# NikNazarov/TorchPIV

Hardware: AMD Instinct MI355X
Metric: image-pairs/sec at 4 MP, wind=64 ov=32 2-pass CWS; % HBM roofline (higher is better)
Workload: dtype u32 exact sums + f64 / f32

## Files before the change

torchpiv_amd/csrc/xcorr_tile.hpp:

```cpp
#pragma once
#include <hip/hip_runtime.h>
#include <stdint.h>
#include <stdlib.h>

#include "fft_inreg.hpp"
#include "piv_kernels.h"

namespace tpiv {

template <int WS, bool PLANAR_ = false>
struct TileGeo {
    static constexpr int WPW = 64 / WS;
    static constexpr int TS = WS > 32 ? 32 : WS;
    static constexpr int PITCH = TS + 1;
    static constexpr int NT = 64 / TS;
    static constexpr int TILE = TS * PITCH;
    static constexpr bool PLANAR = PLANAR_;
    static constexpr int HROWS = WS / 2 + 1;
    static constexpr int HTILE = HROWS * PITCH;
    static constexpr int LDS_FLOATS = NT * TILE * (PLANAR ? 1 : 2);
    static constexpr int MAP_PITCH = WS + 1;
    static constexpr int NDW = WS / 4;
};

// ... 84 lines not shown
template <int K, int N>
__device__ __forceinline__ float byte_f(const uint32_t (&d)[N]) {
    return (float)((d[K >> 2] >> (8 * (K & 3))) & 0xffu);
}

#ifndef TPIV_SDWA_LERP
#define TPIV_SDWA_LERP 0
#endif
constexpr float SDWA_UP = 0x1p125f, SDWA_DN = 0x1p-24f, SDWA_INV = 0x1p24f;
template <int K, int N>
__device__ __forceinline__ float byte_d(const uint32_t (&d)[N]) {
    return __uint_as_float((d[K >> 2] >> (8 * (K & 3))) & 0xffu);
}

template <int N>
__device__ __forceinline__ void load_dwords(const uint8_t* __restrict__ p, uint32_t (&d)[N]) {
    __builtin_memcpy(&d[0], p, 4 * N);
}

__device__ __forceinline__ float bilerp_ref(float f11, float f21, float f12, float f22, float wx_up,
                                            float wx_dn, float wy_up, float wy_dn, bool degenerate) {
#pragma clang fp contract(off)
    float r = (f11 * wx_up) * wy_up;
    r = r + (f21 * wx_dn) * wy_up;
    r = r + (f12 * wx_up) * wy_dn;
    r = r + (f22 * wx_dn) * wy_dn;
    return degenerate ? f11 : r;
}

__device__ __forceinline__ float bilerp_ref_m(float f11, float f21, float f12, float f22, float wx_up,
                                              float wx_dn, float wy_up, float wy_dn, unsigned degenerate_mask) {
#pragma clang fp contract(off)
    float r = (f11 * wx_up) * wy_up;
    r = r + (f21 * wx_dn) * wy_up;
    r = r + (f12 * wx_up) * wy_dn;
    r = r + (f22 * wx_dn) * wy_dn;
    const unsigned bits = (degenerate_mask & __float_as_uint(f11)) | (~degenerate_mask & __float_as_uint(r));
    return __uint_as_float(bits);
}

#ifdef TPIV_STAMPS
#define TPIV_STAMP_DECL unsigned long long st_acc[16] = {}; unsigned long long st_prev = 0; unsigned st_iter = 0; \
    unsigned long long st_t0 = __builtin_amdgcn_s_memtime(), st_r0 = __builtin_amdgcn_s_memrealtime();
#define TPIV_STAMP_START                                                                  \
    do {                                                                                  \
        __builtin_amdgcn_sched_barrier(0);                                                \
        asm volatile("s_memtime %0\n\ts_waitcnt lgkmcnt(0)" : "=s"(st_prev)::"memory");    \
        __builtin_amdgcn_sched_barrier(0);                                                \
    } while (0)
#define TPIV_STAMP(i)                                                                     \
    do {                                                                                  \
        unsigned long long st_t;                                                          \
        __builtin_amdgcn_sched_barrier(0);                                                \
        asm volatile("s_memtime %0\n\ts_waitcnt lgkmcnt(0)" : "=s"(st_t)::"memory");       \
        __builtin_amdgcn_sched_barrier(0);                                                \
        st_acc[i] += st_t - st_prev;                                                      \
        st_prev = st_t;                                                                   \
    } while (0)
#define TPIV_STAMP_FLUSH(pp)                                                              \
    do {                                                                                  \
        if ((pp).stamps != nullptr && threadIdx.x == 0) {                                 \
            for (int q_ = 0; q_ < 16; ++q_) atomicAdd(&(pp).stamps[q_], st_acc[q_]);      \
            atomicAdd(&(pp).stamps[16], (unsigned long long)st_iter);                     \
            atomicAdd(&(pp).stamps[17], __builtin_amdgcn_s_memtime() - st_t0);            \
            atomicAdd(&(pp).stamps[18], __builtin_amdgcn_s_memrealtime() - st_r0);        \
        }                                                                                 \
    } while (0)
#else
#define TPIV_STAMP_DECL
#define TPIV_STAMP_START
#define TPIV_STAMP(i)
#define TPIV_STAMP_FLUSH(pp)
#endif

__device__ __forceinline__ int fast_div(int n, unsigned magic, int shift) {
    return (int)(((unsigned long long)(unsigned)n * magic) >> shift);
}
inline void fast_div_setup(unsigned d, unsigned& magic, int& shift) {
    int s_ = 0;
    while ((1ull << s_) < d) ++s_;
    shift = 31 + s_;
    magic = (unsigned)(((1ull << shift) + d - 1) / d);
}

__device__ __forceinline__ int fresh_lane() {
    int l = (int)__builtin_amdgcn_mbcnt_hi(~0u, __builtin_amdgcn_mbcnt_lo(~0u, 0u));
    asm volatile("" : "+v"(l));
    return l;
}

__device__ __forceinline__ void wave_sync() {
    __builtin_amdgcn_fence(__ATOMIC_ACQ_REL, "wavefront");
    __builtin_amdgcn_wave_barrier();
}

template <int WS, bool DIGITREV, bool PLANAR>
__device__ __forceinline__ void transpose_tile(cf (&a)[WS], float* lds, int lane) {
    using G = TileGeo<WS, PLANAR>;
    constexpr int P = G::PITCH;
    cf* tile = reinterpret_cast<cf*>(lds);
    if constexpr (PLANAR && WS > 32) {
        static_for<0, 32>([&](auto kc) TPIV_LAMBDA_INLINE {
            constexpr int k = decltype(kc)::value;
            constexpr int lo = DIGITREV ? FFT_POS<k, WS> : k;
            constexpr int hi = DIGITREV ? FFT_POS<k + 32, WS> : k + 32;
            auto rx = __builtin_amdgcn_permlane32_swap(__float_as_uint(a[lo].x), __float_as_uint(a[hi].x),
                                                       false, false);
            auto ry = __builtin_amdgcn_permlane32_swap(__float_as_uint(a[lo].y), __float_as_uint(a[hi].y),
                                                       false, false);
            a[lo].x = __uint_as_float(rx[0]);
            a[hi].x = __uint_as_float(rx[1]);
            a[lo].y = __uint_as_float(ry[0]);
            a[hi].y = __uint_as_float(ry[1]);
        });
        float* t = lds + (lane >> 5) * G::TILE;
        const int i = lane & 31;
        auto plane = [&](auto comp) TPIV_LAMBDA_INLINE {
            constexpr bool Y = decltype(comp)::value;
            float lowhalf[32];
            wave_sync();
            static_for<0, 32>([&](auto kc) TPIV_LAMBDA_INLINE {
                constexpr int k = decltype(kc)::value;
                constexpr int src = DIGITREV ? FFT_POS<k, WS> : k;
                t[i * P + k] = Y ? a[src].y : a[src].x;
            });
            wave_sync();
#pragma unroll
            for (int r = 0; r < 32; ++r) lowhalf[r] = t[r * P + i];
            wave_sync();
            static_for<0, 32>([&](auto kc) TPIV_LAMBDA_INLINE {
                constexpr int k = decltype(kc)::value;
                constexpr int src = DIGITREV ? FFT_POS<k + 32, WS> : k + 32;
                t[i * P + k] = Y ? a[src].y : a[src].x;
            });
            wave_sync();
#pragma unroll
            for (int r = 0; r < 32; ++r) {
                if constexpr (Y) {
                    a[32 + r].y = t[r * P + i];
                    a[r].y = lowhalf[r];
                } else {
                    a[32 + r].x = t[r * P + i];
                    a[r].x = lowhalf[r];
                }
            }
        };
        plane(std::false_type{});
        plane(std::true_type{});
    } else if constexpr (PLANAR) {
        float* t = lds + (lane / WS) * G::TILE;
        const int i = lane % WS;
        wave_sync();
        static_for<0, WS>([&](auto kc) TPIV_LAMBDA_INLINE {
            constexpr int k = decltype(kc)::value;
            constexpr int src = DIGITREV ? FFT_POS<k, WS> : k;
            t[i * P + k] = a[src].x;
        });
        wave_sync();
#pragma unroll
        for (int r = 0; r < WS; ++r) a[r].x = t[r * P + i];
        wave_sync();
        static_for<0, WS>([&](auto kc) TPIV_LAMBDA_INLINE {
            constexpr int k = decltype(kc)::value;
            constexpr int src = DIGITREV ? FFT_POS<k, WS> : k;
            t[i * P + k] = a[src].y;
        });
        wave_sync();
#pragma unroll
        for (int r = 0; r < WS; ++r) a[r].y = t[r * P + i];
    } else if constexpr (WS <= 32) {
        cf* t = tile + (lane / WS) * G::TILE;
        const int i = lane % WS;
        wave_sync();
        static_for<0, WS>([&](auto kc) TPIV_LAMBDA_INLINE {
            constexpr int k = decltype(kc)::value;
            constexpr int src = DIGITREV ? FFT_POS<k, WS> : k;
            t[i * P + k] = a[src];
        });
        wave_sync();
#pragma unroll
        for (int r = 0; r < WS; ++r) a[r] = t[r * P + i];
    } else {
        static_for<0, 32>([&](auto kc) TPIV_LAMBDA_INLINE {
            constexpr int k = decltype(kc)::value;
            constexpr int lo = DIGITREV ? FFT_POS<k, WS> : k;
            constexpr int hi = DIGITREV ? FFT_POS<k + 32, WS> : k + 32;
            auto rx = __builtin_amdgcn_permlane32_swap(__float_as_uint(a[lo].x), __float_as_uint(a[hi].x),
                                                       false, false);
            auto ry = __builtin_amdgcn_permlane32_swap(__float_as_uint(a[lo].y), __float_as_uint(a[hi].y),
                                                       false, false);
            a[lo].x = __uint_as_float(rx[0]);
            a[hi].x = __uint_as_float(rx[1]);
            a[lo].y = __uint_as_float(ry[0]);
            a[hi].y = __uint_as_float(ry[1]);
        });
        cf* t = tile + (lane >> 5) * G::TILE;
        const int i = lane & 31;
        cf lowhalf[32];
        wave_sync();
        static_for<0, 32>([&](auto kc) TPIV_LAMBDA_INLINE {
            constexpr int k = decltype(kc)::value;
            constexpr int src = DIGITREV ? FFT_POS<k, WS> : k;
            t[i * P + k] = a[src];
        });
        wave_sync();
#pragma unroll
        for (int r = 0; r < 32; ++r) lowhalf[r] = t[r * P + i];
        wave_sync();
        static_for<0, 32>([&](auto kc) TPIV_LAMBDA_INLINE {
            constexpr int k = decltype(kc)::value;
            constexpr int src = DIGITREV ? FFT_POS<k + 32, WS> : k + 32;
            t[i * P + k] = a[src];
        });
        wave_sync();
#pragma unroll
        for (int r = 0; r < 32; ++r) a[32 + r] = t[r * P + i];
#pragma unroll
        for (int r = 0; r < 32; ++r) a[r] = lowhalf[r];
    }
}

template <int WS, bool PLANAR>
__device__ __forceinline__ void transpose_half(const cf (&a)[WS], cf (&g)[WS / 2 + 1], float* lds, int lane) {
    static_assert(WS <= 32 || WS == 64, "one tile per window");
    using G = TileGeo<WS, PLANAR>;
    constexpr int P = G::PITCH, M = WS / 2;
    const int i = lane % WS;
    if constexpr (WS == 64) {
        constexpr int Q = M + 1;
        static_assert(WS * Q * (PLANAR ? 1 : 2) <= G::LDS_FLOATS, "half-spectrum plane fits the tile");
        cf b[WS];
        static_for<0, WS>([&](auto kc) TPIV_LAMBDA_INLINE {
            constexpr int k = decltype(kc)::value;
            b[k] = a[FFT_POS<k, WS>];
            asm volatile("" : "+v"(b[k].x), "+v"(b[k].y));
        });
        wave_sync();
        if constexpr (!PLANAR) {
            cf* t = reinterpret_cast<cf*>(lds);
            if (i <= M) {
                static_for<0, WS>([&](auto kc) TPIV_LAMBDA_INLINE {
                    constexpr int k = decltype(kc)::value;
                    t[k * Q + i] = b[k];
                });
            }
            wave_sync();
#pragma unroll
            for (int r = 0; r <= M; ++r) g[r] = t[i * Q + r];
        } else {
        if (i <= M) {
            static_for<0, WS>([&](auto kc) TPIV_LAMBDA_INLINE {
                constexpr int k = decltype(kc)::value;
                lds[k * Q + i] = b[k].x;
            });
        }
        wave_sync();
#pragma unroll
        for (int r = 0; r <= M; ++r) g[r].x = lds[i * Q + r];
        wave_sync();
        if (i <= M) {
            static_for<0, WS>([&](auto kc) TPIV_LAMBDA_INLINE {
                constexpr int k = decltype(kc)::value;
                lds[k * Q + i] = b[k].y;
            });
        }
        wave_sync();
#pragma unroll
        for (int r = 0; r <= M; ++r) g[r].y = lds[i * Q + r];
        }
    } else if constexpr (PLANAR) {
        float* t = lds + (lane / WS) * G::HTILE;
        wave_sync();
        if (i <= M) {
            static_for<0, WS>([&](auto kc) TPIV_LAMBDA_INLINE {
                constexpr int k = decltype(kc)::value;
                t[i * P + k] = a[FFT_POS<k, WS>].x;
            });
        }
        wave_sync();
#pragma unroll
        for (int r = 0; r <= M; ++r) g[r].x = t[r * P + i];
        wave_sync();
        if (i <= M) {
            static_for<0, WS>([&](auto kc) TPIV_LAMBDA_INLINE {
                constexpr int k = decltype(kc)::value;
                t[i * P + k] = a[FFT_POS<k, WS>].y;
            });
        }
        wave_sync();
#pragma unroll
        for (int r = 0; r <= M; ++r) g[r].y = t[r * P + i];
    } else {
        cf* t = reinterpret_cast<cf*>(lds) + (lane / WS) * G::HTILE;
        wave_sync();
        if (i <= M) {
            static_for<0, WS>([&](auto kc) TPIV_LAMBDA_INLINE {
                constexpr int k = decltype(kc)::value;
                t[i * P + k] = a[FFT_POS<k, WS>];
            });
        }
        wave_sync();
#pragma unroll
        for (int r = 0; r <= M; ++r) g[r] = t[r * P + i];
    }
}

struct ItemGeom {
    int pair, win, y0, x0;
    int active;
    size_t fidx;
};

#ifndef TPIV_COOP1
#define TPIV_COOP1 0
#endif
template <int WS>
struct Coop1 {
    static constexpr bool ON = TPIV_COOP1 && (WS == 64 || WS == 32);
    static constexpr int P16 = WS / 16;
    static constexpr int PITCH4 = WS / 16 + 1;
};
template <int WS, int MODE>
struct RawRows;
template <int WS>
struct RawRows<WS, MODE_PASS1> {
    uint32_t a[WS / 4], b[WS / 4];
};
template <int WS>
struct RawRows<WS, MODE_DWS> {
    uint32_t a[WS / 4], b[WS / 4];
    long long qa, qb;
    int reg;
    int cls;
    int fix;
};
template <int WS>
struct CoopGeo {
#ifndef TPIV_COOP
#define TPIV_COOP 1
#endif
    static constexpr bool ON = TPIV_COOP && (WS == 16 || WS == 32 || WS == 64);
    static constexpr int NROW = WS + 1;
    static constexpr int RPG = (WS + 1 + 15) / 16;
    static constexpr int LOADED = 16 * RPG;
    static constexpr int T = NROW * RPG;
    static constexpr int NCH = (T + WS - 1) / WS;
    static constexpr int PITCH4 = RPG | 1;
    static constexpr int PATCH4 = NROW * PITCH4;
    static constexpr int BLOCK4 = (2 * PATCH4 + 15) / 16 * 16;
    static constexpr int FLOATS = (64 / WS) * BLOCK4 * 4;
    static constexpr int LDS_FLOATS = FLOATS + (64 / WS) * (WS + 1) * 4;
    static_assert(!ON || RPG <= PITCH4, "patch row pitch");
    __device__ static __forceinline__ void chunk(int ci, int& j, int& part) {
        if constexpr (RPG == 2) {
            j = ci >> 1;
            part = ci & 1;
        } else if constexpr (RPG == 3) {
            j = (ci * 171) >> 9;
            part = ci - 3 * j;
        } else {
            static_assert(RPG == 5, "chunks per row");
            j = (ci * 205) >> 10;
            part = ci - 5 * j;
        }
    }
};
template <int WS>
struct CoopOff {
    int o[CoopGeo<WS>::ON ? CoopGeo<WS>::NCH : 1];
    __device__ __forceinline__ void init(int r, int W) {
        if constexpr (CoopGeo<WS>::ON) {
#pragma unroll
            for (int k = 0; k < CoopGeo<WS>::NCH; ++k) {
                int j, part;
                CoopGeo<WS>::chunk(r + WS * k, j, part);
                o[k] = r + WS * k < CoopGeo<WS>::T ? j * W + 16 * part : 0;
            }
        }
    }
};
template <int WS>
struct RawRows<WS, MODE_CWS> {
    static constexpr int NB = WS / 4 + 1;
    uint32_t a0[CoopGeo<WS>::ON ? 1 : NB], a1[CoopGeo<WS>::ON ? 1 : NB], b0[CoopGeo<WS>::ON ? 1 : NB], b1[CoopGeo<WS>::ON ? 1 : NB];
    uint32_t ca[CoopGeo<WS>::ON ? CoopGeo<WS>::NCH : 1][4], cb[CoopGeo<WS>::ON ? CoopGeo<WS>::NCH : 1][4];
    int reg;
    int cls;
    int fix;
};

struct CwsRow {
    float wya_up, wya_dn, wyb_up, wyb_dn;
    int dya, uya, dyb, uyb;
    int ydeg_a, ydeg_b;
};
__device__ __forceinline__ CwsRow cws_row(int gy, float vy) {
    CwsRow c;
    const float gyf = (float)gy;
    const float nya = gyf - vy, nyb = gyf + vy;
    const float uya_f = ceilf(nya), dya_f = floorf(nya);
    const float uyb_f = ceilf(nyb), dyb_f = floorf(nyb);
    c.uya = f2i_sat_t(uya_f);
    c.dya = f2i_sat_t(dya_f);
    c.uyb = f2i_sat_t(uyb_f);
    c.dyb = f2i_sat_t(dyb_f);
    c.wya_up = uya_f - nya;
    c.wya_dn = nya - dya_f;
    c.wyb_up = uyb_f - nyb;
    c.wyb_dn = nyb - dyb_f;
    c.ydeg_a = c.uya == c.dya;
    c.ydeg_b = c.uyb == c.dyb;
    return c;
}

__device__ __forceinline__ int classify_row(long long q, int used, int loaded, int HW, long long& qload) {
    const long long lim = (long long)HW - loaded;
    if (q >= 0 && q <= lim) {
        qload = q;
        return 0;
    }
    if (q + used - 1 <= 0) {
        qload = 0;
        return 1;
    }
    if (q >= (long long)HW - 1) {
        qload = lim;
        return 2;
    }
    qload = 0;
    return 3;
}

__device__ __forceinline__ int clamp_i(int v, int lo, int hi) { return v < lo ? lo : (v > hi ? hi : v); }

__device__ __forceinline__ int classify_row32(int q, int used, int loaded, int HW, int& qload) {
    const int lim = HW - loaded;
    const bool inside = (unsigned)q <= (unsigned)lim;
    const bool before = q + used - 1 <= 0;
    const bool behind = q >= HW - 1;
    qload = inside ? q : (behind && !before ? lim : 0);
    return inside ? 0 : (before ? 1 : (behind ? 2 : 3));
}

template <int N>
__device__ __forceinline__ void fix_row(uint32_t (&d)[N], int cls) {
    const uint32_t px = (cls == 1 ? (d[0] & 0xffu) : (d[N - 1] >> 24)) * 0x01010101u;
#pragma unroll
    for (int i = 0; i < N; ++i) d[i] = cls != 0 ? px : d[i];
}
template <int N>
__device__ __forceinline__ void fix_row(uint32_t (&d)[N], int cls, uint32_t last) {
    const uint32_t px = (cls == 1 ? (d[0] & 0xffu) : (last >> 24)) * 0x01010101u;
#pragma unroll
    for (int i = 0; i < N; ++i) d[i] = cls != 0 ? px : d[i];
}

template <int WS, int MODE, bool FAST = false>
__device__ __forceinline__ void issue_rows(const PassParams& p, const ItemGeom& g, int r, float vx, float vy,
                                           RawRows<WS, MODE>& raw, const CoopOff<WS>& coff) {
    const int HW = p.H * p.W;
    const uint8_t* __restrict__ fa = p.A + (size_t)g.pair * HW;
    const uint8_t* __restrict__ fb = p.B + (size_t)g.pair * HW;
    const long long base = (long long)(g.y0 + r) * p.W + g.x0;
    if constexpr (MODE == MODE_PASS1) {
        if constexpr (Coop1<WS>::ON) {
            using C1 = Coop1<WS>;
            const unsigned o0 = (unsigned)(g.y0 * p.W + g.x0);
#pragma unroll
            for (int k = 0; k < C1::P16; ++k) {
                const int ci = r + WS * k, j = ci / C1::P16, part = ci % C1::P16;
                const unsigned o_ = o0 + (unsigned)(j * p.W + 16 * part);
                load_dwords<4>(fa + o_, *reinterpret_cast<uint32_t(*)[4]>(&raw.a[4 * k]));
                load_dwords<4>(fb + o_, *reinterpret_cast<uint32_t(*)[4]>(&raw.b[4 * k]));
            }
        } else {
#ifdef TPIV_EXP_P1LOADS
            load_dwords<4 * TPIV_EXP_P1LOADS>(fa + base, *reinterpret_cast<uint32_t(*)[4 * TPIV_EXP_P1LOADS]>(&raw.a[0]));
            load_dwords<4 * TPIV_EXP_P1LOADS>(fb + base, *reinterpret_cast<uint32_t(*)[4 * TPIV_EXP_P1LOADS]>(&raw.b[0]));
#pragma unroll
            for (int k = 4 * TPIV_EXP_P1LOADS; k < WS / 4; ++k) {
                raw.a[k] = 0x11213141u * (unsigned)(r + 1 + k);
                raw.b[k] = 0x31112141u * (unsigned)(r + 3 + k);
            }
#else
            load_dwords<WS / 4>(fa + base, raw.a);
            load_dwords<WS / 4>(fb + base, raw.b);
#endif
        }
    } else if constexpr (MODE == MODE_DWS) {
        const long long sh = (long long)vy * p.W + (long long)vx;
        raw.qa = base - sh;
        raw.qb = base + sh;
        long long la, lb;
        const int ca = classify_row(raw.qa, WS, WS, HW, la), cb = classify_row(raw.qb, WS, WS, HW, lb);
        raw.reg = __all(ca != 3 && cb != 3) ? 1 : 0;
        raw.cls = ca | (cb << 2);
        raw.fix = (raw.reg && __any(raw.cls != 0)) ? 1 : 0;
        load_dwords<WS / 4>(fa + (raw.reg ? la : base), raw.a);
        load_dwords<WS / 4>(fb + (raw.reg ? lb : base), raw.b);
    } else {
        constexpr int NB = WS / 4 + 1;
        const CwsRow c = cws_row(g.y0 + r, vy);
        const float fvx = floorf(vx);
        const int W_ = p.W;
        const int ivx = clamp_i(f2i_sat_t(fvx), -W_, W_);
        const int rlo = -8, rhi = p.H + 7;
        const int dya = clamp_i(c.dya, rlo, rhi), uya = clamp_i(c.uya, rlo, rhi);
        const int dyb = clamp_i(c.dyb, rlo, rhi), uyb = clamp_i(c.uyb, rlo, rhi);
        const int xa = g.x0 - ivx - 1, xb = g.x0 + ivx;
        const int qa0 = dya * W_ + xa, qa1 = uya * W_ + xa;
        const int qb0 = dyb * W_ + xb, qb1 = uyb * W_ + xb;
        using CG = CoopGeo<WS>;
        constexpr int LOADED = CG::ON ? CG::LOADED : 4 * NB;
        const float gxr = (float)(g.x0 + r);
        const float nxa_r = gxr - vx, nxb_r = gxr + vx;
        const float fxa_r = floorf(nxa_r), fxb_r = floorf(nxb_r);
        const bool col_ok = fxa_r == (float)(g.x0 + r - ivx - 1) && fxb_r == (float)(g.x0 + r + ivx) &&
                            fxa_r != nxa_r && fxb_r != nxb_r;
        bool reg = col_ok && fabsf(vx) < (float)p.W && !(FAST && (c.ydeg_a | c.ydeg_b));
        int la0 = 0, la1 = 0, lb0 = 0, lb1 = 0, cls = 0;
        auto classify_own = [&]() TPIV_LAMBDA_INLINE {
            const int c0 = classify_row32(qa0, WS + 1, LOADED, HW, la0), c1 = classify_row32(qa1, WS + 1, LOADED, HW, la1);
            const int c2 = classify_row32(qb0, WS + 1, LOADED, HW, lb0), c3 = classify_row32(qb1, WS + 1, LOADED, HW, lb1);
            reg = reg && c0 != 3 && c1 != 3 && c2 != 3 && c3 != 3;
            cls = c0 | (c1 << 2) | (c2 << 4) | (c3 << 6);
        };
        if constexpr (CG::ON) {
            const float gy0f = (float)g.y0;
            const int base_a = clamp_i(f2i_sat_t(floorf(gy0f - vy)), rlo, rhi);
            const int base_b = clamp_i(f2i_sat_t(floorf(gy0f + vy)), rlo, rhi);
            reg = reg && (unsigned)(dya - base_a) <= (unsigned)WS && (unsigned)(uya - base_a) <= (unsigned)WS &&
                  (unsigned)(dyb - base_b) <= (unsigned)WS && (unsigned)(uyb - base_b) <= (unsigned)WS;
            const bool inside = base_a >= 0 && base_a + WS < p.H && base_b >= 0 && base_b + WS < p.H &&
                                xa >= 0 && xa + LOADED <= W_ && xb >= 0 && xb + LOADED <= W_;
            const bool all_in = __all(inside);
            if (!all_in) classify_own();
            raw.reg = __all(reg) ? 1 : 0;
            raw.cls = cls;
            raw.fix = (raw.reg && __any(raw.cls != 0)) ? 1 : 0;
            unsigned oa[CG::NCH], ob[CG::NCH];
            if (all_in) {
                const int qa_o = base_a * W_ + xa, qb_o = base_b * W_ + xb;
#pragma unroll
                for (int k = 0; k < CG::NCH; ++k) {
                    oa[k] = (unsigned)(qa_o + coff.o[k]);
                    ob[k] = (unsigned)(qb_o + coff.o[k]);
                }
            } else {
#pragma unroll
                for (int k = 0; k < CG::NCH; ++k) {
                    const int ci = r + WS * k;
                    int j, part;
                    CG::chunk(ci, j, part);
                    int qa_l, qb_l;
                    const int ra = clamp_i(base_a + j, rlo, rhi), rb = clamp_i(base_b + j, rlo, rhi);
                    classify_row32(ra * W_ + xa, WS + 1, LOADED, HW, qa_l);
                    classify_row32(rb * W_ + xb, WS + 1, LOADED, HW, qb_l);
                    const bool live = ci < CG::T;
                    oa[k] = live ? (unsigned)(qa_l + 16 * part) : 0u;
                    ob[k] = live ? (unsigned)(qb_l + 16 * part) : 0u;
                }
            }
#pragma unroll
            for (int k = 0; k < CG::NCH; ++k) {
                load_dwords<4>(fa + oa[k], raw.ca[k]);
                load_dwords<4>(fb + ob[k], raw.cb[k]);
            }
        } else {
        classify_own();
        raw.reg = __all(reg) ? 1 : 0;
        raw.cls = cls;
        raw.fix = (raw.reg && __any(raw.cls != 0)) ? 1 : 0;
        const int lim = HW - 4 * NB;
        const int base32 = (g.y0 + r) * W_ + g.x0;
        const int safe = base32 < lim ? base32 : lim;
        load_dwords<NB>(fa + (unsigned)(raw.reg ? la0 : safe), raw.a0);
        load_dwords<NB>(fa + (unsigned)(raw.reg ? la1 : safe), raw.a1);
        load_dwords<NB>(fb + (unsigned)(raw.reg ? lb0 : safe), raw.b0);
        load_dwords<NB>(fb + (unsigned)(raw.reg ? lb1 : safe), raw.b1);
        }
    }
}

__device__ __forceinline__ uint32_t read_unit_x(const uint4* src) {
    uint4 t = *src;
    asm volatile("" : "+v"(t.x), "+v"(t.y), "+v"(t.z), "+v"(t.w));
    return t.x;
}

struct RowSquares {
    unsigned aa, bb;
};
template <int WS, int MODE, int RBH = 1, bool FAST = false, bool SQ = false, int PATH = 0>
__device__ __forceinline__ void convert_rows(const PassParams& p, const ItemGeom& g, int r, int lane, float vx,
                                             float vy, RawRows<WS, MODE>& raw, cf (&x)[WS], float& sa,
                                             float& sb, float* lds, RowSquares* sq = nullptr) {
    const int HW = p.H * p.W;
    const uint8_t* __restrict__ fa = p.A + (size_t)g.pair * HW;
    const uint8_t* __restrict__ fb = p.B + (size_t)g.pair * HW;
    static constexpr int RBL = WS / RBH;
    float* rowbuf = lds + lane * (RBL + 1);
    static constexpr int UNR_DWS = WS <= 16 ? 1 : 4, UNR_CWS = WS <= 16 ? 1 : 2;
    if constexpr (MODE == MODE_PASS1) {
        if constexpr (Coop1<WS>::ON) {
            using C1 = Coop1<WS>;
            uint4* const t4 = reinterpret_cast<uint4*>(lds) + (lane / WS) * (WS * C1::PITCH4);
// ... 427 lines not shown
#pragma unroll
            for (int k = 0; k < WS; ++k) my_row[(k + WS / 2) % WS] = row[k];
        }
        wave_sync();
        return my_row[r];
    };
    auto row_of_lane = [](int rl) TPIV_LAMBDA_INLINE { return (rl + WS / 2) % WS; };
    int m = 0;
    {
        const unsigned long long rows = wballot(rmax >= gmax - band);
        open = open || __popcll(rows) != 1;
        const int rl = rows ? (int)__builtin_ctzll(rows) : 0;
        const unsigned long long cols = wballot(park(rl) >= gmax - band);
        open = open || __popcll(cols) != 1;
        m = row_of_lane(rl) * WS + (cols ? (int)__builtin_ctzll(cols) : 0);
    }
    const int wv = p.val_win;
    int s[EXACT_MAX_SECOND] = {-1, -1, -1};
    {
        const unsigned long long ex = exclusion_row_mask<WS>(m, ys, wv);
        const int exl = (int)(unsigned)ex, exh = (int)(unsigned)(ex >> 32);
        int smax = -1;
        static_for<0, WS>([&](auto kc) TPIV_LAMBDA_INLINE {
            constexpr int xsft = decltype(kc)::value;
            constexpr int xo = (xsft + WS / 2) % WS;
            const int kill = __builtin_amdgcn_sbfe(xsft < 32 ? exl : exh, xsft & 31, 1);
            const int cnd = __float_as_int(__fsub_rn(row[xo], cmin)) | kill;
            smax = cnd > smax ? cnd : smax;
        });
        const int sall = grp_reduce<WS>(smax, [](int a, int b) TPIV_LAMBDA_INLINE { return a > b ? a : b; });
        const float thr = __int_as_float(sall) - band;
        unsigned long long rows = sall >= 0 ? wballot(smax >= 0 && __int_as_float(smax) >= thr) : 0ull;
        open = open || __popcll(rows) > EXACT_MAX_SECOND;
        int ns = 0;
        for (int it = 0; it < EXACT_MAX_SECOND; ++it) {
            if (!any_left(rows)) break;
            const bool on = mine_left(rows);
            const int rl = on ? (int)__builtin_ctzll(rows) : 0;
            rows &= rows - 1;
            const int yr = row_of_lane(rl);
            const unsigned long long exr = exclusion_row_mask<WS>(m, yr, wv);
            unsigned long long cols = wballot(__fsub_rn(park(rl), cmin) >= thr) & ~exr;
            cols = on ? cols : 0ull;
            for (int k = 0; k < WS; ++k) {
                if (!any_left(cols)) break;
                const bool has = mine_left(cols);
                const int q = yr * WS + (has ? (int)__builtin_ctzll(cols) : 0);
                cols &= cols - 1;
                s[0] = (has && ns == 0) ? q : s[0];
                s[1] = (has && ns == 1) ? q : s[1];
                s[2] = (has && ns == 2) ? q : s[2];
                ns += has ? 1 : 0;
            }
        }
        open = open || ns > EXACT_MAX_SECOND;
    }
    int n[EXACT_MAX_MIN] = {-1, -1, -1, -1};
    {
        const float thr = cmin + band;
        unsigned long long rows = wballot(rmin <= thr);
        bool over = __popcll(rows) > EXACT_MAX_MIN;
        int nn = 0;
        for (int it = 0; it < EXACT_MAX_MIN; ++it) {
            if (!any_left(rows)) break;
            const bool on = mine_left(rows);
            const int rl = on ? (int)__builtin_ctzll(rows) : 0;
            rows &= rows - 1;
            const int yr = row_of_lane(rl);
            unsigned long long cols = wballot(park(rl) <= thr);
            cols = on ? cols : 0ull;
            over = over || nn + __popcll(cols) > EXACT_MAX_MIN;
            for (int k = 0; k < EXACT_MAX_MIN; ++k) {
                if (!any_left(cols)) break;
                const bool has = mine_left(cols) && cols != 0ull && nn < EXACT_MAX_MIN;
                const int q = yr * WS + (cols ? (int)__builtin_ctzll(cols) : 0);
                cols &= cols - 1;
                n[0] = (has && nn == 0) ? q : n[0];
                n[1] = (has && nn == 1) ? q : n[1];
                n[2] = (has && nn == 2) ? q : n[2];
                n[3] = (has && nn == 3) ? q : n[3];
                nn += has ? 1 : 0;
            }
        }
        n[3] = over ? -2 : n[3];
    }
    if (r == 0 && active) {
        const int m_out = dead ? -2 : (open ? -1 : m);
        auto pack = [](int lo_, int hi_) TPIV_LAMBDA_INLINE { return ((unsigned)lo_ & 0xffffu) | ((unsigned)hi_ << 16); };
        uint4 rec;
        rec.x = pack(m_out, s[0]);
        rec.y = pack(s[1], s[2]);
        rec.z = pack(n[0], n[1]);
        rec.w = pack(n[2], n[3]);
        p.cand[fidx] = rec;
    }
}

template <int WS, int MODE, int OCC, bool FAST, bool CAND, int ROLE = 0>
__device__ __forceinline__ void xcorr_tile_body(const PassParams& p) {
    constexpr bool PLANAR = OCC > 2;
    using G = TileGeo<WS, PLANAR>;
    static_assert(WS == 8 || WS == 16 || WS == 32 || WS == 64, "tile sizes of this kernel");
    constexpr int RBH = 64 * (WS + 1) <= G::LDS_FLOATS ? 1 : 2;
    static_assert(MODE == MODE_PASS1 || 64 * (WS / RBH + 1) <= G::LDS_FLOATS,
                  "slow-path row buffer (shifted passes) must fit the tile LDS");
    constexpr int LDSF = (MODE == MODE_CWS && CoopGeo<WS>::ON && CoopGeo<WS>::LDS_FLOATS > G::LDS_FLOATS)
                             ? CoopGeo<WS>::LDS_FLOATS : G::LDS_FLOATS;
    __shared__ __attribute__((aligned(16))) float tile[LDSF];

#ifndef TPIV_TWREG32
#define TPIV_TWREG32 0
#endif
    using TW = std::conditional_t<((WS == 32 && TPIV_TWREG32) || WS == 16), TwRegs<WS>, TwLiteral>;
    TW tw;
    if constexpr (!std::is_same<TW, TwLiteral>::value) tw.init();

    const int N = p.n_rows * p.n_cols;
    const int groups = (N + G::WPW - 1) / G::WPW;
    const bool listed = ROLE == 0 && MODE != MODE_PASS1 && p.list_mode != 0;
    const int items = listed ? __builtin_amdgcn_readfirstlane((int)*p.slow_count) : p.batch * groups;
    const int st = p.ws - p.ov;
    auto real_item = [&](int pos) TPIV_LAMBDA_INLINE { return listed ? __builtin_amdgcn_readfirstlane(p.slow_list[pos]) : pos; };

    constexpr int QCH = WS <= 16 ? 4 : 1;
    const int xcd = blockIdx.x & 7;
    const int chunk = (int)(((long long)items + 7) / 8);
    const int lo = __builtin_amdgcn_readfirstlane(xcd * chunk < items ? xcd * chunk : items);
    const int hi = __builtin_amdgcn_readfirstlane(items - lo > chunk ? lo + chunk : items);
    unsigned* const ctr = p.work_ctr + xcd * 16;
    int q_base = 0;
    int q_left = 0;
    auto q_issue = [&]() TPIV_LAMBDA_INLINE -> unsigned {
        unsigned v = 0;
        if (QCH == 1 || q_left == 0) {
            if (fresh_lane() == 0) v = atomicAdd(ctr, (unsigned)QCH);
        }
        return v;
    };
    auto q_take = [&](unsigned q_raw) TPIV_LAMBDA_INLINE -> int {
        if (QCH == 1 || q_left == 0) {
            const unsigned v = (unsigned)__builtin_amdgcn_readfirstlane((int)q_raw);
            q_base = v < (unsigned)(hi - lo) ? lo + (int)v : hi;
            q_left = QCH;
        }
        const int it = q_base + (QCH - q_left);
        --q_left;
        return it;
    };

    auto geom_of = [&](int pos, int w) TPIV_LAMBDA_INLINE {
        ItemGeom g;
        const int item = real_item(pos);
        g.pair = fast_div(item, p.groups_magic, p.groups_shift);
        const int gi = item - g.pair * groups;
        const int win_raw = gi * G::WPW + w;
        g.active = win_raw < N ? 1 : 0;
        g.win = g.active ? win_raw : N - 1;
        const int wrow = fast_div(g.win, p.ncols_magic, p.ncols_shift);
        g.y0 = wrow * st;
        g.x0 = (g.win - wrow * p.n_cols) * st;
        g.fidx = (size_t)g.pair * N + g.win;
        return g;
    };
    auto shift_of = [&](const ItemGeom& g, float& vx, float& vy) TPIV_LAMBDA_INLINE {
        if constexpr (MODE == MODE_PASS1) {
            vx = 0.f;
            vy = 0.f;
        } else {
            if constexpr (MODE == MODE_CWS) {
                pred_half_shift_cws_f32(p, g.fidx, vx, vy);
            } else {
                double sx, sy;
                pred_half_shift<MODE>(p, g.fidx, sx, sy);
                vx = (float)sx;
                vy = (float)sy;
            }
        }
    };

    int item = q_take(q_issue());
    if (item >= hi) return;
    int nitem = q_take(q_issue());
    constexpr bool RECOMPUTE = WS >= 32;
    float vx, vy;
    RawRows<WS, MODE> raw;
    ItemGeom gcur;
    CoopOff<WS> coff;
    if constexpr (MODE == MODE_CWS) coff.init(fresh_lane() % WS, p.W);
    {
        const int l0 = fresh_lane();
        gcur = geom_of(item, l0 / WS);
        shift_of(gcur, vx, vy);
        issue_rows<WS, MODE, FAST>(p, gcur, l0 % WS, vx, vy, raw, coff);
    }

    TPIV_STAMP_DECL
    TPIV_STAMP_START;
    for (int nnitem; item < hi; item = nitem, nitem = nnitem) {
        const unsigned q_raw = q_issue();
#ifdef TPIV_STAMPS
        ++st_iter;
#endif
        const int lane = fresh_lane();
        const int w = lane / WS;
        const int r = lane % WS;
        const ItemGeom g = RECOMPUTE ? geom_of(item, w) : gcur;
        const bool active = g.active != 0;
        const size_t fidx = g.fidx;
        const int nit = nitem < hi ? nitem : item;
        const ItemGeom gnext = geom_of(nit, w);
        float nvx, nvy;
        shift_of(gnext, nvx, nvy);

        if constexpr (ROLE == 1) {
            if (!raw.reg) {
                if (lane == 0) p.slow_list[atomicAdd(p.slow_count, 1u)] = item;
                nnitem = q_take(q_raw);
                issue_rows<WS, MODE, FAST>(p, gnext, r, nvx, nvy, raw, coff);
                vx = nvx;
                vy = nvy;
                if constexpr (!RECOMPUTE) gcur = gnext;
                continue;
            }
        }
        cf x[WS];
        float sa, sb;
        constexpr int NBS = WS >= 32 ? G::WPW : 1;
        int band_s[NBS];
        TPIV_STAMP(0);
        RowSquares sq;
        convert_rows<WS, MODE, RBH, FAST, CAND, ROLE == 1 ? 1 : 0>(p, g, r, lane, vx, vy, raw, x, sa, sb, tile, &sq);
        TPIV_STAMP(1);
        if constexpr (WS >= 64) nnitem = q_take(q_raw);
        if constexpr (WS <= 32) issue_rows<WS, MODE, FAST>(p, gnext, r, nvx, nvy, raw, coff);

        if (p.dbg_win != nullptr && active) {
            int rr = r;
            asm volatile("" : "+v"(rr));
            float* d = p.dbg_win + fidx * 2 * WS * WS + rr * WS;
            constexpr float UNS = (MODE == MODE_CWS && FAST && TPIV_SDWA_LERP) ? SDWA_INV : 1.0f;
#pragma unroll
            for (int k = 0; k < WS; ++k) {
                d[k] = x[k].x * UNS;
                d[WS * WS + k] = x[k].y * UNS;
            }
        }

        bool dead = false;
        float end_scale = 1.0f;
        constexpr bool FASTN = FAST && MODE != MODE_PASS1;
        if constexpr (!FASTN) {
            sa = grp_sum<WS>(sa);
            sb = grp_sum<WS>(sb);
            const float ma = sa * (1.0f / (WS * WS)), mb = sb * (1.0f / (WS * WS));
            float ka = 1.f, kb = 1.f;
            if constexpr (MODE == MODE_PASS1) {
                dead = (sa == 0.f) || (sb == 0.f);
                ka = dead ? 0.f : 1.0f / ma;
                kb = dead ? 0.f : 1.0f / mb;
            }
            if constexpr (CAND) {
                auto uadd = [](unsigned a_, unsigned b_) TPIV_LAMBDA_INLINE { return a_ + b_; };
                const unsigned saa = grp_reduce<WS>(sq.aa, uadd), sbb = grp_reduce<WS>(sq.bb, uadd);
                constexpr double NN = (double)(WS * WS);
                const double da = (double)sa, db = (double)sb;
                const float ea = (float)__fma_rn(-da, da, NN * (double)saa), eb = (float)__fma_rn(-db, db, NN * (double)sbb);
                const float e_plus = (0.5f / (float)(WS * WS)) * (ea * (ka * ka) + eb * (kb * kb));
                const float bnd = dead ? 0.f : p.exact_band * e_plus;
                if constexpr (WS >= 32) {
                    static_for<0, G::WPW>([&](auto wc) TPIV_LAMBDA_INLINE {
                        band_s[decltype(wc)::value] = __builtin_amdgcn_readlane(__float_as_int(bnd), decltype(wc)::value * WS);
                    });
                } else {
                    band_s[0] = __float_as_int(bnd);
                }
            }
            constexpr float PRE = 0.5f / (float)WS;
            const float oa = -ma * ka, ob = -mb * kb;
            const float kas = ka * PRE, kbs = kb * PRE, oas = oa * PRE, obs = ob * PRE;
#pragma unroll
            for (int k = 0; k < WS; ++k) {
                x[k].x = fmaf(x[k].x, kas, oas);
                x[k].y = fmaf(x[k].y, kbs, obs);
            }
        }

        TPIV_STAMP(2);
        fft_inreg<WS, 1>(x, tw);
        if constexpr (FASTN) {
            constexpr int P0 = FFT_POS<0, WS>;
            const float ta = grp_sum<WS>(x[P0].x);
            const float tb = grp_sum<WS>(x[P0].y);
            x[P0].x -= ta * (1.0f / WS);
            x[P0].y -= tb * (1.0f / WS);
            end_scale = 0.25f / (float)(WS * WS);
            if constexpr (MODE == MODE_CWS && TPIV_SDWA_LERP) end_scale *= SDWA_INV * SDWA_INV;
        }
        TPIV_STAMP(3);
        transpose_tile<WS, true, PLANAR>(x, tile, fresh_lane());
        TPIV_STAMP(4);
        fft_inreg<WS, 1>(x, tw);
        TPIV_STAMP(5);

        {
            const int lane_c = fresh_lane();
            const int r_c = lane_c % WS;
            const int partner = (lane_c - r_c) + ((WS - r_c) % WS);
            auto cross = [&](cf zk, cf zm) TPIV_LAMBDA_INLINE {
                const float a_ = zk.x, b_ = zk.y, c_ = zm.x, d_ = zm.y;
                cf pr;
                pr.x = (a_ * d_ + b_ * c_) * 2.0f;
                pr.y = (c_ * c_ - a_ * a_) + (d_ * d_ - b_ * b_);
                return pr;
            };
            static_for<0, WS / 2 + 1>([&](auto kc) TPIV_LAMBDA_INLINE {
                constexpr int ky = decltype(kc)::value;
                constexpr int nky = (WS - ky) % WS;
                constexpr int p1 = FFT_POS<ky, WS>, p2 = FFT_POS<nky, WS>;
                const cf z1 = x[p1];
                if constexpr (ky == nky) {
                    cf m1;
                    m1.x = __shfl(z1.x, partner, 64);
                    m1.y = __shfl(z1.y, partner, 64);
                    x[p1] = cross(z1, m1);
                } else {
                    const cf z2 = x[p2];
                    cf m1, m2;
                    m1.x = __shfl(z2.x, partner, 64);
                    m1.y = __shfl(z2.y, partner, 64);
                    m2.x = __shfl(z1.x, partner, 64);
                    m2.y = __shfl(z1.y, partner, 64);
                    x[p1] = cross(z1, m1);
                    x[p2] = cross(z2, m2);
                }
            });
        }

        TPIV_STAMP(6);
        cf t[WS];
        static_for<0, WS>([&](auto kc) TPIV_LAMBDA_INLINE {
            constexpr int ky = decltype(kc)::value;
            t[ky] = x[FFT_POS<ky, WS>];
        });
        fft_inreg<WS, -1>(t, tw);
        TPIV_STAMP(7);
#ifndef TPIV_C2R
#define TPIV_C2R 1
#endif
        float crow[WS];
#ifndef TPIV_C2R64
#define TPIV_C2R64 1
#endif
        if constexpr (TPIV_C2R && (WS <= 32 || (TPIV_C2R64 && WS == 64))) {
            cf hs[WS / 2 + 1], z[WS / 2];
            transpose_half<WS, PLANAR>(t, hs, tile, fresh_lane());
            TPIV_STAMP(8);
            c2r_inreg<WS>(hs, z);
            static_for<0, WS>([&](auto xc) TPIV_LAMBDA_INLINE {
                constexpr int x_ = decltype(xc)::value;
                crow[x_] = (x_ & 1) ? z[FFT_POS<x_ / 2, WS / 2>].y : z[FFT_POS<x_ / 2, WS / 2>].x;
            });
        } else {
            transpose_tile<WS, true, PLANAR>(t, tile, fresh_lane());
            TPIV_STAMP(8);
            fft_inreg<WS, -1>(t, tw);
            static_for<0, WS>([&](auto xc) TPIV_LAMBDA_INLINE {
                constexpr int x_ = decltype(xc)::value;
                crow[x_] = t[FFT_POS<x_, WS>].x;
            });
        }
        wave_sync();
        TPIV_STAMP(9);

        auto band_of = [&](int w_) TPIV_LAMBDA_INLINE {
            int b_ = band_s[0];
            static_for<1, NBS>([&](auto wc) TPIV_LAMBDA_INLINE { b_ = w_ == decltype(wc)::value ? band_s[decltype(wc)::value] : b_; });
            return __int_as_float(b_);
        };
        if constexpr (WS > 32) {
            const int lane_p = fresh_lane();
            issue_rows<WS, MODE, FAST>(p, geom_of(nit, lane_p / WS), lane_p % WS, nvx, nvy, raw, coff);
        }
        vx = nvx;
        vy = nvy;
        if constexpr (!RECOMPUTE) gcur = gnext;

        TPIV_STAMP(10);
        if constexpr (RECOMPUTE) {
            const int lane_e = fresh_lane();
            const int w_e = lane_e / WS, r_e = lane_e % WS;
            const int item_e = real_item(item);
            const int pair_e = fast_div(item_e, p.groups_magic, p.groups_shift);
            const int win_raw_e = (item_e - pair_e * groups) * G::WPW + w_e;
            const bool active_e = win_raw_e < N;
            const int win_e = active_e ? win_raw_e : N - 1;
            const size_t fidx_e = (size_t)pair_e * N + win_e;
            if constexpr (CAND) peak_candidates<WS>(p, crow, tile, w_e, r_e, active_e, dead, fidx_e, band_of(w_e));
            else peak_analysis<WS, PLANAR, FASTN>(p, crow, tile, w_e, r_e, active_e, dead, fidx_e, end_scale);
        } else {
            if constexpr (CAND) peak_candidates<WS>(p, crow, tile, w, r, active, dead, fidx, band_of(w));
            else peak_analysis<WS, PLANAR, FASTN>(p, crow, tile, w, r, active, dead, fidx, end_scale);
        }
        wave_sync();
        if constexpr (WS < 64) nnitem = q_take(q_raw);
        TPIV_STAMP(13);
    }
    TPIV_STAMP_FLUSH(p);
}

template <int WS, int MODE, int OCC, bool FAST>
__global__ __launch_bounds__(64, OCC) void xcorr_tile_kernel(PassParams p) {
    xcorr_tile_body<WS, MODE, OCC, FAST, false>(p);
}
template <int WS, int MODE>
__global__ __launch_bounds__(64, 3) void xcorr_tile_fastpath_kernel(PassParams p) {
    xcorr_tile_body<WS, MODE, 3, true, false, 1>(p);
}
template <int WS>
__global__ __launch_bounds__(64, tile_occ_c(WS, MODE_PASS1)) void xcorr_tile_cand_kernel(PassParams p) {
    xcorr_tile_body<WS, MODE_PASS1, tile_occ_c(WS, MODE_PASS1), true, true>(p);
}

template <int WS, bool PLANAR>
__global__ __launch_bounds__(64, 2) void peak_debug_kernel(PassParams p, const float* maps, int n_maps) {
    using G = TileGeo<WS, PLANAR>;
    __shared__ float tile[G::LDS_FLOATS];
    const int lane = threadIdx.x;
    const int w = lane / WS, r = lane % WS;
    const int win_raw = blockIdx.x * G::WPW + w;
    const bool active = win_raw < n_maps;
    const int win = active ? win_raw : n_maps - 1;
    float crow[WS];
    const int ys = (r + WS / 2) % WS;
#pragma unroll
    for (int xo = 0; xo < WS; ++xo) crow[xo] = maps[((size_t)win * WS + ys) * WS + (xo + WS / 2) % WS];
    peak_analysis<WS, PLANAR>(p, crow, tile, w, r, active, false, (size_t)win);
}

template <int WS>
hipError_t launch_peak_debug(const PassParams& p, const float* maps, int n_maps, int planar, hipStream_t stream) {
    using G = TileGeo<WS, false>;
    const int blocks = (n_maps + G::WPW - 1) / G::WPW;
    if (planar)
        hipLaunchKernelGGL((peak_debug_kernel<WS, true>), dim3(blocks), dim3(64), 0, stream, p, maps, n_maps);
    else
        hipLaunchKernelGGL((peak_debug_kernel<WS, false>), dim3(blocks), dim3(64), 0, stream, p, maps, n_maps);
    return hipGetLastError();
}

template <int WS, int MODE>
static hipError_t launch_tile(const PassParams& p_in, int n_cu, hipStream_t stream) {
    using G = TileGeo<WS>;
    PassParams p = p_in;
    const int N = p.n_rows * p.n_cols;
    const long long groups = (N + G::WPW - 1) / G::WPW;
    const long long items = (long long)p.batch * groups;
    if (items <= 0 || items >= (1ll << 31) - 64) return hipErrorInvalidValue;
    fast_div_setup((unsigned)groups, p.groups_magic, p.groups_shift);
    fast_div_setup((unsigned)p.n_cols, p.ncols_magic, p.ncols_shift);
    long long blocks = items;
    static const int wg_per_cu = [] {
        const char* e = getenv("TPIV_WG_PER_CU");
        return e ? atoi(e) : 0;
    }();
    const long long cap = (long long)n_cu * (wg_per_cu > 0 ? wg_per_cu : 64);
    if (blocks > cap) blocks = cap;
    blocks = (blocks + 7) / 8 * 8;
    constexpr int OCC = tile_occ_c(WS, MODE);
    if constexpr (MODE != MODE_PASS1) {
        if (p.precision != 0) {
            hipLaunchKernelGGL((xcorr_tile_kernel<WS, MODE, OCC, false>), dim3((unsigned)blocks), dim3(64), 0, stream, p);
            return hipGetLastError();
        }
    }
#ifdef TPIV_EXPERIMENT
    static const int occ_env = [] {
        const char* e = getenv("TPIV_OCC");
        return e ? atoi(e) : 0;
    }();
    if (occ_env == 2 && OCC != 2) {
        hipLaunchKernelGGL((xcorr_tile_kernel<WS, MODE, 2, true>), dim3((unsigned)blocks), dim3(64), 0, stream, p);
        return hipGetLastError();
    }
    if constexpr (WS <= 32 || MODE != MODE_CWS) {
        if (occ_env == 3 && OCC != 3) {
            hipLaunchKernelGGL((xcorr_tile_kernel<WS, MODE, 3, true>), dim3((unsigned)blocks), dim3(64), 0, stream, p);
            return hipGetLastError();
        }
    }
    if constexpr (WS <= 32) {
        if (occ_env == 4 && OCC != 4) {
            hipLaunchKernelGGL((xcorr_tile_kernel<WS, MODE, 4, true>), dim3((unsigned)blocks), dim3(64), 0, stream, p);
            return hipGetLastError();
        }
    }
#endif
    if constexpr (tile_split64(WS, MODE)) {
        if (p.slow_list != nullptr && p.slow_count != nullptr) {
            hipLaunchKernelGGL((xcorr_tile_fastpath_kernel<WS, MODE>), dim3((unsigned)blocks), dim3(64), 0, stream, p);
            hipError_t e_ = hipGetLastError();
            if (e_ != hipSuccess) return e_;
            e_ = hipMemsetAsync(p.work_ctr, 0, TILE_CTR_BYTES, stream);
            if (e_ != hipSuccess) return e_;
            PassParams q = p;
            q.list_mode = 1;
            long long blocks2 = (long long)n_cu * 8;
            if (blocks2 > blocks) blocks2 = blocks;
            blocks2 = (blocks2 + 7) / 8 * 8;
            hipLaunchKernelGGL((xcorr_tile_kernel<WS, MODE, OCC, true>), dim3((unsigned)blocks2), dim3(64), 0, stream, q);
            return hipGetLastError();
        }
    }
    hipLaunchKernelGGL((xcorr_tile_kernel<WS, MODE, OCC, true>), dim3((unsigned)blocks), dim3(64), 0, stream, p);
    return hipGetLastError();
}

template <int WS>
hipError_t launch_xcorr_tile_cand_ws(const PassParams& p_in, int n_cu, hipStream_t stream) {
    using G = TileGeo<WS>;
    PassParams p = p_in;
    const int N = p.n_rows * p.n_cols;
    const long long groups = (N + G::WPW - 1) / G::WPW;
    const long long items = (long long)p.batch * groups;
    if (items <= 0 || items >= (1ll << 31) - 64 || p.cand == nullptr) return hipErrorInvalidValue;
    fast_div_setup((unsigned)groups, p.groups_magic, p.groups_shift);
    fast_div_setup((unsigned)p.n_cols, p.ncols_magic, p.ncols_shift);
    long long blocks = items < (long long)n_cu * 64 ? items : (long long)n_cu * 64;
    blocks = (blocks + 7) / 8 * 8;
    hipLaunchKernelGGL((xcorr_tile_cand_kernel<WS>), dim3((unsigned)blocks), dim3(64), 0, stream, p);
    return hipGetLastError();
}

template <int WS>
hipError_t launch_xcorr_tile_ws(const PassParams& p, int mode, int n_cu, hipStream_t stream) {
    switch (mode) {
        case MODE_PASS1: return launch_tile<WS, MODE_PASS1>(p, n_cu, stream);
        case MODE_DWS: return launch_tile<WS, MODE_DWS>(p, n_cu, stream);
        case MODE_CWS: return launch_tile<WS, MODE_CWS>(p, n_cu, stream);
        default: return hipErrorInvalidValue;
    }
}

}
```

Before: 16590.

## Use half-length inverse FFT on Hermitian cross-spectrum with paired-row transpose

For planar 32/64 tiles, the cross-spectrum product is built for only the half spectrum. Each column is then packed into a complex sequence of length WS/2 using a real-signal twiddle post-step, so the first inverse pass runs an FFT of length WS/2 instead of WS. A new transpose_half_pairs routine rebuilds the half-spectrum rows through LDS in two planar passes, ahead of the existing C2R stage. This is meant to cut inverse-FFT arithmetic and register pressure, at the cost of extra shuffles, sign handling and an additional LDS round trip.

After: 17660, median of 6. +6.5%, better.

```diff
diff --git a/torchpiv_amd/csrc/xcorr_tile.hpp b/torchpiv_amd/csrc/xcorr_tile.hpp
--- a/torchpiv_amd/csrc/xcorr_tile.hpp
+++ b/torchpiv_amd/csrc/xcorr_tile.hpp
@@ -410,6 +410,55 @@
         wave_sync();
 #pragma unroll
         for (int r = 0; r <= M; ++r) g[r] = t[r * P + i];
+    }
+}
+
+template <int WS, bool PLANAR>
+__device__ __forceinline__ void transpose_half_pairs(const cf (&h)[WS / 2], cf (&g)[WS / 2 + 1], float* lds, int lane) {
+    static_assert(PLANAR && (WS == 32 || WS == 64), "planar tiles of 32 and 64");
+    using G = TileGeo<WS, PLANAR>;
+    constexpr int M = WS / 2, Q = M + 1;
+    static_assert(64 * Q <= G::LDS_FLOATS, "the half-spectrum plane fits the tile");
+    const int r = lane % WS;
+    float* t = lds + (lane / WS) * (WS * Q);
+    const bool odd = r > M;
+    constexpr bool ZERO_ODD = WS == 32;
+    const bool up = odd || (r == 0 && ZERO_ODD) || (r == M && !ZERO_ODD);
+    float* wp = t + (odd ? WS - r : r) + (up ? Q : 0);
+    const float sy = odd ? -1.0f : 1.0f;
+    cf b[M];
+    static_for<0, M>([&](auto mc) TPIV_LAMBDA_INLINE {
+        constexpr int m = decltype(mc)::value;
+        b[m] = h[FFT_POS<m, M>];
+        asm volatile("" : "+v"(b[m].x), "+v"(b[m].y));
+    });
+    const int y = lane % WS;
+    const float* rd = t + y * Q;
+    const float* r0 = t + ((y & ~1) + (ZERO_ODD ? 1 : 0)) * Q;
+    const float* rm = t + ((y & ~1) + (ZERO_ODD ? 0 : 1)) * Q + M;
+    wave_sync();
+    static_for<0, M>([&](auto mc) TPIV_LAMBDA_INLINE {
+        constexpr int m = decltype(mc)::value;
+        wp[2 * Q * m] = b[m].x;
+    });
+    wave_sync();
+    g[0].x = r0[0];
+#pragma unroll
+    for (int k = 1; k < M; ++k) g[k].x = rd[k];
+    g[M].x = rm[0];
+    wave_sync();
+    static_for<0, M>([&](auto mc) TPIV_LAMBDA_INLINE {
+        constexpr int m = decltype(mc)::value;
+        wp[2 * Q * m] = b[m].y * sy;
+    });
+    wave_sync();
+    g[0].y = r0[0];
+#pragma unroll
+    for (int k = 1; k < M; ++k) g[k].y = rd[k];
+    g[M].y = rm[0];
+    if (y & 1) {
+        g[0].x = g[0].y;
+        g[M].x = g[M].y;
     }
 }
 
@@ -1443,72 +1492,130 @@
         fft_inreg<WS, 1>(x, tw);
         TPIV_STAMP(5);
 
-        {
-            const int lane_c = fresh_lane();
-            const int r_c = lane_c % WS;
-            const int partner = (lane_c - r_c) + ((WS - r_c) % WS);
-            auto cross = [&](cf zk, cf zm) TPIV_LAMBDA_INLINE {
-                const float a_ = zk.x, b_ = zk.y, c_ = zm.x, d_ = zm.y;
-                cf pr;
-                pr.x = (a_ * d_ + b_ * c_) * 2.0f;
-                pr.y = (c_ * c_ - a_ * a_) + (d_ * d_ - b_ * b_);
-                return pr;
-            };
-            static_for<0, WS / 2 + 1>([&](auto kc) TPIV_LAMBDA_INLINE {
-                constexpr int ky = decltype(kc)::value;
-                constexpr int nky = (WS - ky) % WS;
-                constexpr int p1 = FFT_POS<ky, WS>, p2 = FFT_POS<nky, WS>;
-                const cf z1 = x[p1];
-                if constexpr (ky == nky) {
-                    cf m1;
-                    m1.x = __shfl(z1.x, partner, 64);
-                    m1.y = __shfl(z1.y, partner, 64);
-                    x[p1] = cross(z1, m1);
-                } else {
-                    const cf z2 = x[p2];
-                    cf m1, m2;
-                    m1.x = __shfl(z2.x, partner, 64);
-                    m1.y = __shfl(z2.y, partner, 64);
-                    m2.x = __shfl(z1.x, partner, 64);
-                    m2.y = __shfl(z1.y, partner, 64);
-                    x[p1] = cross(z1, m1);
-                    x[p2] = cross(z2, m2);
-                }
-            });
-        }
-
-        TPIV_STAMP(6);
-        cf t[WS];
-        static_for<0, WS>([&](auto kc) TPIV_LAMBDA_INLINE {
-            constexpr int ky = decltype(kc)::value;
-            t[ky] = x[FFT_POS<ky, WS>];
-        });
-        fft_inreg<WS, -1>(t, tw);
-        TPIV_STAMP(7);
 #ifndef TPIV_C2R
 #define TPIV_C2R 1
 #endif
-        float crow[WS];
 #ifndef TPIV_C2R64
 #define TPIV_C2R64 1
 #endif
-        if constexpr (TPIV_C2R && (WS <= 32 || (TPIV_C2R64 && WS == 64))) {
-            cf hs[WS / 2 + 1], z[WS / 2];
-            transpose_half<WS, PLANAR>(t, hs, tile, fresh_lane());
+#ifndef TPIV_HALF_INV64
+#define TPIV_HALF_INV64 1
+#endif
+#ifndef TPIV_HALF_INV32
+#define TPIV_HALF_INV32 1
+#endif
+        constexpr bool HALF_INV = PLANAR && TPIV_C2R &&
+                                  ((WS == 64 && TPIV_C2R64 && TPIV_HALF_INV64) || (WS == 32 && TPIV_HALF_INV32));
+        float crow[WS];
+        if constexpr (HALF_INV) {
+            constexpr int M = WS / 2;
+            cf h[M];
+            {
+                const int lane_c = fresh_lane();
+                const int r_c = lane_c % WS;
+                const int partner = (lane_c - r_c) + ((WS - r_c) % WS);
+                auto cross = [&](cf zk, cf zm) TPIV_LAMBDA_INLINE {
+                    const float a_ = zk.x, b_ = zk.y, c_ = zm.x, d_ = zm.y;
+                    cf pr;
+                    pr.x = (a_ * d_ + b_ * c_) * 2.0f;
+                    pr.y = (c_ * c_ - a_ * a_) + (d_ * d_ - b_ * b_);
+                    return pr;
+                };
+                cf pc[M + 1];
+                static_for<0, M + 1>([&](auto kc) TPIV_LAMBDA_INLINE {
+                    constexpr int ky = decltype(kc)::value;
+                    constexpr int nky = (WS - ky) % WS;
+                    const cf z2 = x[FFT_POS<nky, WS>];
+                    cf m1;
+                    m1.x = __shfl(z2.x, partner, 64);
+                    m1.y = __shfl(z2.y, partner, 64);
+                    pc[ky] = cross(x[FFT_POS<ky, WS>], m1);
+                });
+                TPIV_STAMP(6);
+                const bool odd = r_c > M;
+                const float fs = (r_c == 0 || r_c == M) ? 1.0f : 0.0f;
+                static_for<0, M>([&](auto kc) TPIV_LAMBDA_INLINE {
+                    constexpr int k = decltype(kc)::value;
+                    cf pr;
+                    pr.x = __shfl(pc[M - k].x, partner, 64);
+                    pr.y = __shfl(pc[M - k].y, partner, 64);
+                    const cf s{pc[k].x + pr.x, pc[k].y - pr.y};
+                    const cf tt = twmul<k, WS, -1>(cf{pc[k].x - pr.x, pc[k].y + pr.y});
+                    h[k].x = odd ? tt.x : __builtin_fmaf(-fs, tt.y, s.x);
+                    h[k].y = odd ? tt.y : __builtin_fmaf(fs, tt.x, s.y);
+                });
+            }
+            fft_inreg<M, -1>(h, tw);
+            TPIV_STAMP(7);
+            cf hs[M + 1], z[M];
+            transpose_half_pairs<WS, PLANAR>(h, hs, tile, fresh_lane());
             TPIV_STAMP(8);
             c2r_inreg<WS>(hs, z);
             static_for<0, WS>([&](auto xc) TPIV_LAMBDA_INLINE {
                 constexpr int x_ = decltype(xc)::value;
-                crow[x_] = (x_ & 1) ? z[FFT_POS<x_ / 2, WS / 2>].y : z[FFT_POS<x_ / 2, WS / 2>].x;
+                crow[x_] = (x_ & 1) ? z[FFT_POS<x_ / 2, M>].y : z[FFT_POS<x_ / 2, M>].x;
             });
         } else {
-            transpose_tile<WS, true, PLANAR>(t, tile, fresh_lane());
-            TPIV_STAMP(8);
+            {
+                const int lane_c = fresh_lane();
+                const int r_c = lane_c % WS;
+                const int partner = (lane_c - r_c) + ((WS - r_c) % WS);
+                auto cross = [&](cf zk, cf zm) TPIV_LAMBDA_INLINE {
+                    const float a_ = zk.x, b_ = zk.y, c_ = zm.x, d_ = zm.y;
+                    cf pr;
+                    pr.x = (a_ * d_ + b_ * c_) * 2.0f;
+                    pr.y = (c_ * c_ - a_ * a_) + (d_ * d_ - b_ * b_);
+                    return pr;
+                };
+                static_for<0, WS / 2 + 1>([&](auto kc) TPIV_LAMBDA_INLINE {
+                    constexpr int ky = decltype(kc)::value;
+                    constexpr int nky = (WS - ky) % WS;
+                    constexpr int p1 = FFT_POS<ky, WS>, p2 = FFT_POS<nky, WS>;
+                    const cf z1 = x[p1];
+                    if constexpr (ky == nky) {
+                        cf m1;
+                        m1.x = __shfl(z1.x, partner, 64);
+                        m1.y = __shfl(z1.y, partner, 64);
+                        x[p1] = cross(z1, m1);
+                    } else {
+                        const cf z2 = x[p2];
+                        cf m1, m2;
+                        m1.x = __shfl(z2.x, partner, 64);
+                        m1.y = __shfl(z2.y, partner, 64);
+                        m2.x = __shfl(z1.x, partner, 64);
+                        m2.y = __shfl(z1.y, partner, 64);
+                        x[p1] = cross(z1, m1);
+                        x[p2] = cross(z2, m2);
+                    }
+                });
+            }
+
+            TPIV_STAMP(6);
+            cf t[WS];
+            static_for<0, WS>([&](auto kc) TPIV_LAMBDA_INLINE {
+                constexpr int ky = decltype(kc)::value;
+                t[ky] = x[FFT_POS<ky, WS>];
+            });
             fft_inreg<WS, -1>(t, tw);
-            static_for<0, WS>([&](auto xc) TPIV_LAMBDA_INLINE {
-                constexpr int x_ = decltype(xc)::value;
-                crow[x_] = t[FFT_POS<x_, WS>].x;
-            });
+            TPIV_STAMP(7);
+            if constexpr (TPIV_C2R && (WS <= 32 || (TPIV_C2R64 && WS == 64))) {
+                cf hs[WS / 2 + 1], z[WS / 2];
+                transpose_half<WS, PLANAR>(t, hs, tile, fresh_lane());
+                TPIV_STAMP(8);
+                c2r_inreg<WS>(hs, z);
+                static_for<0, WS>([&](auto xc) TPIV_LAMBDA_INLINE {
+                    constexpr int x_ = decltype(xc)::value;
+                    crow[x_] = (x_ & 1) ? z[FFT_POS<x_ / 2, WS / 2>].y : z[FFT_POS<x_ / 2, WS / 2>].x;
+                });
+            } else {
+                transpose_tile<WS, true, PLANAR>(t, tile, fresh_lane());
+                TPIV_STAMP(8);
+                fft_inreg<WS, -1>(t, tw);
+                static_for<0, WS>([&](auto xc) TPIV_LAMBDA_INLINE {
+                    constexpr int x_ = decltype(xc)::value;
+                    crow[x_] = t[FFT_POS<x_, WS>].x;
+                });
+            }
         }
         wave_sync();
         TPIV_STAMP(9);
```
